# BICLab/Spike2Former

Measured on AMD Instinct MI355X. Metric: fwd+bwd images/sec, 512x512 T=4 ADE20K-150, higher is better.
Workload: dtype f32 (fp32-equivalent: bf16 hi+mid+lo split operands on bf16 MFMA, fp32 accumulate; spike maps stored as bf16, exact); 1 GPU; C2: 512x512 T=4 K=150 Meta-SpikeFormer [64, 128, 256, 360] + MaskFormer head, per-GPU batch 2; global_batch=2, parallelism=dp1, weights=random-init (name-seeded)

## Files before the change

spike2former_amd/csrc/dwconv.hip:

```cpp
#include "s2f_common.h"
#include <cstdlib>

#pragma clang fp contract(fast)

namespace {

constexpr int TS = 32;

__device__ __forceinline__ float ldx(const float* p) { return *p; }
__device__ __forceinline__ float ldx(const unsigned short* p) { return __uint_as_float(((unsigned int)*p) << 16); }
__device__ __forceinline__ float4 ldx4(const float* p) { return *reinterpret_cast<const float4*>(p); }
__device__ __forceinline__ float4 ldx4(const unsigned short* p) {
  const uint2 v = *reinterpret_cast<const uint2*>(p);
  return make_float4(__uint_as_float(v.x << 16), __uint_as_float(v.x & 0xffff0000u), __uint_as_float(v.y << 16),
                     __uint_as_float(v.y & 0xffff0000u));
}

template <int K, typename TX>
__device__ __forceinline__ void stage_halo(float (&s)[TS + K - 1][TS + K], const TX* __restrict__ xp, int H, int W, int oy0,
                                           int ox0, int po, float fillv, int fpad, bool vec_ok) {
  constexpr int HS = TS + K - 1;
  auto at = [&](int iy, int ix) -> float {
    if (iy >= 0 && iy < H && ix >= 0 && ix < W) return ldx(xp + (int64_t)iy * W + ix);
    if (iy >= -fpad && iy < H + fpad && ix >= -fpad && ix < W + fpad) return fillv;
    return 0.f;
  };
  {
    const int ri = threadIdx.x >> 3, qi = (threadIdx.x & 7) * 4;
    const int iy = oy0 + po + ri, ix = ox0 + po + qi;
    float4 v;
    if (vec_ok && iy >= 0 && iy < H && ix >= 0 && ix + 3 < W) {
      v = ldx4(xp + (int64_t)iy * W + ix);
    } else {
      v = make_float4(at(iy, ix), at(iy, ix + 1), at(iy, ix + 2), at(iy, ix + 3));
    }
    float* d = &s[po + ri][po + qi];
    d[0] = v.x; d[1] = v.y; d[2] = v.z; d[3] = v.w;
  }
  constexpr int RING = HS * HS - TS * TS;
  const int top = po * HS, bot = (K - 1 - po) * HS;
  for (int e = threadIdx.x; e < RING; e += 256) {
    int r, q;
    if (e < top) {
      r = e / HS; q = e - r * HS;
    } else if (e < top + bot) {
      const int f = e - top;
      r = po + TS + f / HS; q = f % HS;
    } else {
      const int f = e - top - bot;
      r = po + f / (K - 1);
      const int j = f % (K - 1);
      q = j < po ? j : TS + j;
    }
    s[r][q] = at(oy0 + r, ox0 + q);
  }
}

struct DwEpi {
  const float* mean;
  const float* var;
  const float* gamma;
  const float* beta;
  float* u_out;
  unsigned short* y;
  unsigned long long* stats;
  float eps, vth, Df, inv_d;
  float* part;
  int P;
};

__device__ __forceinline__ void dw_epi_store(const DwEpi& ep, int c, int64_t off, const float (&acc)[4], int nvalid, bool vec,
                                             uint32_t& csum, uint32_t& cnz) {
#pragma clang fp contract(off)
  const float mean = ep.mean[c], rstd = 1.0f / sqrtf(ep.var[c] + ep.eps), g = ep.gamma[c], be = ep.beta[c];
  float u[4], yy[4] = {0.f, 0.f, 0.f, 0.f};
#pragma unroll
  for (int o = 0; o < 4; ++o) {
    u[o] = (acc[o] - mean) * rstd * g + be;
    if (ep.y && o < nvalid) {
      float sp, vn;
      bool inr;
      s2f_lif_update(u[o], ep.Df, ep.inv_d, ep.vth, sp, yy[o], vn, inr);
      csum += (uint32_t)sp;
      cnz += ((uint32_t)sp != 0);
    }
  }
  if (vec && nvalid == 4) {
    if (ep.u_out) *reinterpret_cast<float4*>(ep.u_out + off) = make_float4(u[0], u[1], u[2], u[3]);
    if (ep.y) *reinterpret_cast<uint2*>(ep.y + off) = s2f_spikes_to_bf16x4(yy[0], yy[1], yy[2], yy[3]);
  } else {
#pragma unroll
    for (int o = 0; o < 4; ++o) {
      if (o >= nvalid) continue;
      if (ep.u_out) ep.u_out[off + o] = u[o];
      if (ep.y) ep.y[off + o] = (unsigned short)(__float_as_uint(yy[o]) >> 16);
    }
  }
}

__device__ __forceinline__ void dw_epi_counters(const DwEpi& ep, uint32_t csum, uint32_t cnz) {
  if (ep.y == nullptr || ep.stats == nullptr) return;
  for (int o = 32; o > 0; o >>= 1) {
    csum += __shfl_xor(csum, o, 64);
    cnz += __shfl_xor(cnz, o, 64);
  }
  if ((threadIdx.x & 63) == 0) {
    unsigned long long* slot = ep.stats + 2 * ((blockIdx.x * 4 + (threadIdx.x >> 6) + blockIdx.y * 7) % S2F_STAT_SLOTS);
    if (csum) atomicAdd(&slot[0], (unsigned long long)csum);
    if (cnz) atomicAdd(&slot[1], (unsigned long long)cnz);
  }
}

__device__ __forceinline__ void dw_tile_stats(const DwEpi& ep, int c, int n, float s1, float s2) {
  __shared__ float red[4][2];
  for (int o = 32; o > 0; o >>= 1) {
    s1 += __shfl_xor(s1, o, 64);
    s2 += __shfl_xor(s2, o, 64);
  }
  if ((threadIdx.x & 63) == 0) {
    red[threadIdx.x >> 6][0] = s1;
    red[threadIdx.x >> 6][1] = s2;
  }
  __syncthreads();
  if (threadIdx.x == 0) {
    const int64_t slot = (int64_t)c * ep.P + (int64_t)n * gridDim.x + blockIdx.x;
    *reinterpret_cast<float2*>(ep.part + slot * 2) =
        make_float2((red[0][0] + red[1][0]) + (red[2][0] + red[3][0]), (red[0][1] + red[1][1]) + (red[2][1] + red[3][1]));
  }
}

template <int K, bool FLIP, typename TX, bool EPI = false, bool STATS = false>
__global__ __launch_bounds__(256) void dw_stencil_kernel(const TX* __restrict__ x, const float* __restrict__ w,
                                                         const float* __restrict__ border, float* __restrict__ y, int C,
                                                         int H, int W, int Ho, int Wo, int pad, int tiles_x, DwEpi ep = DwEpi{}) {
  constexpr int HS = TS + K - 1;
  __shared__ float s[HS][HS + 1];
  const int plane = blockIdx.y;
  const int c = plane % C;
  const int ty = (blockIdx.x / tiles_x) * TS, tx = (blockIdx.x % tiles_x) * TS;
  const TX* xp = x + (int64_t)plane * H * W;
  const float fillv = (!FLIP && border) ? border[c] : 0.f;
  const int po = FLIP ? K - 1 - pad : pad;
  const bool vec_ok = (W & 3) == 0 && (reinterpret_cast<uintptr_t>(xp) & (4 * sizeof(TX) - 1)) == 0;
  stage_halo<K, TX>(s, xp, H, W, ty - po, tx - po, po, fillv, FLIP ? 0 : pad, vec_ok);
  float wk[K * K];
#pragma unroll
  for (int i = 0; i < K * K; ++i) wk[i] = w[c * K * K + i];
  __syncthreads();
  const int r = threadIdx.x >> 3;
  const int q0 = (threadIdx.x & 7) * 4;
  float acc[4] = {0.f, 0.f, 0.f, 0.f};
#pragma unroll
  for (int i = 0; i < K; ++i) {
    float row[K + 3];
#pragma unroll
    for (int j = 0; j < K + 3; ++j) row[j] = s[r + i][q0 + j];
#pragma unroll
    for (int j = 0; j < K; ++j) {
      const float wv = FLIP ? wk[(K - 1 - i) * K + (K - 1 - j)] : wk[i * K + j];
#pragma unroll
      for (int o = 0; o < 4; ++o) acc[o] += wv * row[j + o];
    }
  }
  const int oy = ty + r;
  if constexpr (EPI) {
    uint32_t csum = 0, cnz = 0;
    if (oy < Ho && tx + q0 < Wo) {
      const int64_t off = (int64_t)plane * Ho * Wo + (int64_t)oy * Wo + tx + q0;
      dw_epi_store(ep, c, off, acc, min(4, Wo - tx - q0), (Wo & 3) == 0 && (off & 3) == 0, csum, cnz);
    }
    dw_epi_counters(ep, csum, cnz);
    return;
  }
  if (oy < Ho) {
    float* yp = y + (int64_t)plane * Ho * Wo + (int64_t)oy * Wo + tx + q0;
    if ((Wo & 3) == 0 && tx + q0 + 3 < Wo && (reinterpret_cast<uintptr_t>(yp) & 15u) == 0) {
      *reinterpret_cast<float4*>(yp) = make_float4(acc[0], acc[1], acc[2], acc[3]);
    } else {
#pragma unroll
      for (int o = 0; o < 4; ++o)
        if (tx + q0 + o < Wo) yp[o] = acc[o];
    }
  }
  if constexpr (STATS) {
    float s1 = 0.f, s2 = 0.f;
#pragma unroll
    for (int o = 0; o < 4; ++o)
      if (oy < Ho && tx + q0 + o < Wo) {
        s1 += acc[o];
        s2 += acc[o] * acc[o];
      }
    dw_tile_stats(ep, c, plane / C, s1, s2);
  }
}

constexpr int WT = 64, HT = 32, WS = WT + 8;

template <int K, bool FLIP, typename TX, bool EPI = false, bool STATS = false>
__global__ __launch_bounds__(256) void dw_stencil_wide_kernel(const TX* __restrict__ x, const float* __restrict__ w,
                                                              const float* __restrict__ border, float* __restrict__ y,
                                                              int C, int H, int W, int Ho, int Wo, int pad, int tiles_x,
                                                              DwEpi ep = DwEpi{}) {
  constexpr int HR = HT + K - 1;
  __shared__ __attribute__((aligned(16))) float s[HR][WS];
  const int plane = blockIdx.y;
  const int c = plane % C;
  const int ty = (blockIdx.x / tiles_x) * HT, tx = (blockIdx.x % tiles_x) * WT;
  const TX* xp = x + (int64_t)plane * H * W;
  const float fillv = (!FLIP && border) ? border[c] : 0.f;
  const int po = pad;
  for (int e = threadIdx.x; e < HR * (WS / 4); e += 256) {
    const int r = e / (WS / 4), g = e - r * (WS / 4);
    const int iy = ty - po + r, ix = tx - 4 + g * 4;
    const bool in = iy >= 0 && iy < H && ix >= 0 && ix < W;
    const float4 v = ldx4(xp + (in ? (int64_t)iy * W + ix : 0));
    *reinterpret_cast<float4*>(&s[r][g * 4]) = in ? v : make_float4(fillv, fillv, fillv, fillv);
  }
  float wk[K * K];
#pragma unroll
  for (int i = 0; i < K * K; ++i) wk[i] = w[c * K * K + i];
  __syncthreads();
  const int r2 = (threadIdx.x >> 4) * 2;
  const int q0 = (threadIdx.x & 15) * 4;
  constexpr int SH = 4 - (K - 1) / 2;
  float acc[2][4] = {{0.f, 0.f, 0.f, 0.f}, {0.f, 0.f, 0.f, 0.f}};
#pragma unroll
  for (int i = 0; i < K + 1; ++i) {
    float row[12];
#pragma unroll
    for (int v4 = 0; v4 < 3; ++v4) {
      const float4 t = *reinterpret_cast<const float4*>(&s[r2 + i][q0 + v4 * 4]);
      row[v4 * 4] = t.x; row[v4 * 4 + 1] = t.y; row[v4 * 4 + 2] = t.z; row[v4 * 4 + 3] = t.w;
    }
#pragma unroll
    for (int a = 0; a < 2; ++a) {
      const int ki = i - a;
      if (ki < 0 || ki >= K) continue;
#pragma unroll
      for (int j = 0; j < K; ++j) {
        const float wv = FLIP ? wk[(K - 1 - ki) * K + (K - 1 - j)] : wk[ki * K + j];
#pragma unroll
        for (int o = 0; o < 4; ++o) acc[a][o] += wv * row[j + o + SH];
      }
    }
  }
  if constexpr (EPI) {
    uint32_t csum = 0, cnz = 0;
#pragma unroll
    for (int a = 0; a < 2; ++a) {
      const int oy = ty + r2 + a, ox = tx + q0;
      if (oy >= Ho || ox >= Wo) continue;
      const int64_t off = (int64_t)plane * Ho * Wo + (int64_t)oy * Wo + ox;
      dw_epi_store(ep, c, off, acc[a], min(4, Wo - ox), (Wo & 3) == 0 && (off & 3) == 0, csum, cnz);
    }
    dw_epi_counters(ep, csum, cnz);
    return;
  }
#pragma unroll
  for (int a = 0; a < 2; ++a) {
    const int oy = ty + r2 + a, ox = tx + q0;
    if (oy >= Ho) continue;
    float* yp = y + (int64_t)plane * Ho * Wo + (int64_t)oy * Wo + ox;
    if ((Wo & 3) == 0 && ox + 3 < Wo && (reinterpret_cast<uintptr_t>(yp) & 15u) == 0) {
      *reinterpret_cast<float4*>(yp) = make_float4(acc[a][0], acc[a][1], acc[a][2], acc[a][3]);
    } else {
#pragma unroll
      for (int o = 0; o < 4; ++o)
        if (ox + o < Wo) yp[o] = acc[a][o];
    }
  }
  if constexpr (STATS) {
    float s1 = 0.f, s2 = 0.f;
#pragma unroll
    for (int a = 0; a < 2; ++a)
#pragma unroll
      for (int o = 0; o < 4; ++o)
        if (ty + r2 + a < Ho && tx + q0 + o < Wo) {
          s1 += acc[a][o];
          s2 += acc[a][o] * acc[a][o];
        }
    dw_tile_stats(ep, c, plane / C, s1, s2);
  }
}

template <int K, typename TX>
__global__ __launch_bounds__(256) void dw_wgrad_kernel(const TX* __restrict__ x, const float* __restrict__ border,
                                                       const float* __restrict__ gy, float* __restrict__ gw, int C, int H,
                                                       int W, int Ho, int Wo, int pad, int tiles_x, int ntiles) {
  constexpr int HS = TS + K - 1;
  constexpr int KK = K * K;
  __shared__ float s[HS][HS + 1];
  __shared__ float red[4][KK];
  const int plane = blockIdx.y;
  const int c = plane % C;
  const TX* xp = x + (int64_t)plane * H * W;
  const float* gp = gy + (int64_t)plane * Ho * Wo;
  const float fillv = border ? border[c] : 0.f;
  const bool vec_ok = (W & 3) == 0 && (reinterpret_cast<uintptr_t>(xp) & (4 * sizeof(TX) - 1)) == 0;
  const int r = threadIdx.x >> 3, q0 = (threadIdx.x & 7) * 4;
  float acc[KK];
#pragma unroll
  for (int t = 0; t < KK; ++t) acc[t] = 0.f;
  for (int tile = blockIdx.x; tile < ntiles; tile += gridDim.x) {
    const int ty = (tile / tiles_x) * TS, tx = (tile % tiles_x) * TS;
    __syncthreads();
    stage_halo<K, TX>(s, xp, H, W, ty - pad, tx - pad, pad, fillv, pad, vec_ok);
    float g[4] = {0.f, 0.f, 0.f, 0.f};
    const int oy = ty + r, ox = tx + q0;
    const float* p = gp + (int64_t)oy * Wo + ox;
    if (oy < Ho) {
      if ((Wo & 3) == 0 && ox + 3 < Wo && (reinterpret_cast<uintptr_t>(p) & 15u) == 0) {
        const float4 v = *reinterpret_cast<const float4*>(p);
        g[0] = v.x; g[1] = v.y; g[2] = v.z; g[3] = v.w;
      } else {
#pragma unroll
        for (int o = 0; o < 4; ++o)
          if (ox + o < Wo) g[o] = p[o];
      }
    }
    __syncthreads();
#pragma unroll
    for (int i = 0; i < K; ++i) {
      float row[K + 3];
#pragma unroll
      for (int j = 0; j < K + 3; ++j) row[j] = s[r + i][q0 + j];
#pragma unroll
      for (int j = 0; j < K; ++j)
        acc[i * K + j] += (g[0] * row[j] + g[1] * row[j + 1]) + (g[2] * row[j + 2] + g[3] * row[j + 3]);
    }
  }
  const int lane = threadIdx.x & 63, wave = threadIdx.x >> 6;
#pragma unroll
  for (int t = 0; t < KK; ++t) {
    const float v = s2f_wave_sum_lane63(acc[t]);
    if (lane == 63) red[wave][t] = v;
  }
  __syncthreads();
  if (threadIdx.x < KK) {
    const float t = (red[0][threadIdx.x] + red[1][threadIdx.x]) + (red[2][threadIdx.x] + red[3][threadIdx.x]);
    atomicAdd(gw + c * KK + threadIdx.x, t);
  }
}

int check(const char* who, int N, int C, int H, int W, int K, int pad, int& Ho, int& Wo) {
  S2F_REQUIRE(N > 0 && C > 0 && H > 0 && W > 0, S2F_EINVAL, "%s: bad shape", who);
  S2F_REQUIRE(K == 3 || K == 5 || K == 7, S2F_EINVAL, "%s: kernel size %d not in {3,5,7}", who, K);
  S2F_REQUIRE(pad >= 0 && pad < K, S2F_EINVAL, "%s: bad padding %d", who, pad);
  Ho = H + 2 * pad - K + 1;
  Wo = W + 2 * pad - K + 1;
  S2F_REQUIRE(Ho > 0 && Wo > 0, S2F_EINVAL, "%s: empty output", who);
  S2F_REQUIRE((int64_t)N * C < 65536 * 16, S2F_EINVAL, "%s: too many planes", who);
  return S2F_OK;
}

constexpr int kStencilSizes[] = {3, 5, 7};
template <class F>
void for_stencil_size(int K, const F& launch) {
  s2f_dispatch<kStencilSizes>([&](int k) { return k == K; }, launch);
}

template <typename TX>
void launch_stencil_epi(int K, dim3 grid, hipStream_t s, const TX* x, const float* w, const float* border, int C, int H, int W, int Ho,
                        int Wo, int pad, int tiles_x, DwEpi ep) {
  if (K == 3 && (W & 3) == 0 && W >= 2 * WT && H >= HT && pad == 1 && (reinterpret_cast<uintptr_t>(x) & (4 * sizeof(TX) - 1)) == 0) {
    const int wx = (Wo + WT - 1) / WT, wy = (Ho + HT - 1) / HT;
    hipLaunchKernelGGL((dw_stencil_wide_kernel<3, false, TX, true>), dim3(wx * wy, grid.y), dim3(256), 0, s, x, w, border,
                       (float*)nullptr, C, H, W, Ho, Wo, pad, wx, ep);
    return;
  }
  for_stencil_size(K, [&](auto i) {
    hipLaunchKernelGGL((dw_stencil_kernel<kStencilSizes[i], false, TX, true>), grid, dim3(256), 0, s, x, w, border, (float*)nullptr,
                       C, H, W, Ho, Wo, pad, tiles_x, ep);
  });
}

inline bool wide_form(int K, int H, int W, int pad) {
  static const bool wide_on = !getenv("S2F_DW_NO_WIDE");
  return wide_on && K == 3 && (W & 3) == 0 && W >= 2 * WT && H >= HT && pad == 1;
}

inline int stats_tiles(int H, int W) {
  return wide_form(3, H, W, 1) ? ((W + WT - 1) / WT) * ((H + HT - 1) / HT) : ((W + TS - 1) / TS) * ((H + TS - 1) / TS);
}

template <typename TX>
void launch_stencil_stats(hipStream_t s, const TX* x, const float* w, float* y, float* part, int N, int C, int H, int W) {
  DwEpi ep{};
  ep.part = part;
  ep.P = N * stats_tiles(H, W);
  if (wide_form(3, H, W, 1)) {
    const int wx = (W + WT - 1) / WT, wy = (H + HT - 1) / HT;
    hipLaunchKernelGGL((dw_stencil_wide_kernel<3, false, TX, false, true>), dim3(wx * wy, N * C), dim3(256), 0, s, x, w,
                       (const float*)nullptr, y, C, H, W, H, W, 1, wx, ep);
    return;
  }
  const int tiles_x = (W + TS - 1) / TS, tiles_y = (H + TS - 1) / TS;
  hipLaunchKernelGGL((dw_stencil_kernel<3, false, TX, false, true>), dim3(tiles_x * tiles_y, N * C), dim3(256), 0, s, x, w,
                     (const float*)nullptr, y, C, H, W, H, W, 1, tiles_x, ep);
}

template <bool FLIP, typename TX>
void launch_stencil(int K, dim3 grid, hipStream_t s, const TX* x, const float* w, const float* border, float* y, int C,
                    int H, int W, int Ho, int Wo, int pad, int tiles_x) {
  if (wide_form(K, H, W, pad) && (reinterpret_cast<uintptr_t>(x) & (4 * sizeof(TX) - 1)) == 0) {
    const int wx = (Wo + WT - 1) / WT, wy = (Ho + HT - 1) / HT;
    hipLaunchKernelGGL((dw_stencil_wide_kernel<3, FLIP, TX>), dim3(wx * wy, grid.y), dim3(256), 0, s, x, w, border, y, C, H, W, Ho,
                       Wo, pad, wx, DwEpi{});
    return;
  }
  for_stencil_size(K, [&](auto i) {
    hipLaunchKernelGGL((dw_stencil_kernel<kStencilSizes[i], FLIP, TX>), grid, dim3(256), 0, s, x, w, border, y, C, H, W, Ho, Wo, pad,
                       tiles_x, DwEpi{});
  });
}

}

extern "C" int s2f_dwconv_fwd(const void* x, const float* w, const float* border, float* y, int N, int C, int H, int W,
                              int K, int pad, int x_bf16, void* stream) {
  S2F_REQUIRE(x && w && y, S2F_EINVAL, "s2f_dwconv_fwd: null pointer");
  int Ho, Wo;
  int rc = check("s2f_dwconv_fwd", N, C, H, W, K, pad, Ho, Wo);
  if (rc) return rc;
  const int tiles_x = (Wo + TS - 1) / TS, tiles_y = (Ho + TS - 1) / TS;
  if (x_bf16)
    launch_stencil<false>(K, dim3(tiles_x * tiles_y, N * C), (hipStream_t)stream, reinterpret_cast<const unsigned short*>(x), w,
                          border, y, C, H, W, Ho, Wo, pad, tiles_x);
  else
    launch_stencil<false>(K, dim3(tiles_x * tiles_y, N * C), (hipStream_t)stream, reinterpret_cast<const float*>(x), w, border,
                          y, C, H, W, Ho, Wo, pad, tiles_x);
  return s2f_check_launch("s2f_dwconv_fwd");
}

extern "C" int64_t s2f_dwconv_stats_slots(int N, int H, int W) {
  return (N > 0 && H > 0 && W > 0) ? (int64_t)N * stats_tiles(H, W) : 0;
}

extern "C" int s2f_dwconv_fwd_stats(const void* x, const float* w, float* y, float* partials, int64_t P, int N, int C, int H, int W,
                                    int x_bf16, void* stream) {
  S2F_REQUIRE(x && w && y && partials, S2F_EINVAL, "s2f_dwconv_fwd_stats: null pointer");
  int Ho, Wo;
  int rc = check("s2f_dwconv_fwd_stats", N, C, H, W, 3, 1, Ho, Wo);
  if (rc) return rc;
  S2F_REQUIRE(P == s2f_dwconv_stats_slots(N, H, W), S2F_EINVAL, "s2f_dwconv_fwd_stats: P must be s2f_dwconv_stats_slots(N, H, W)");
  S2F_REQUIRE((reinterpret_cast<uintptr_t>(x) & (x_bf16 ? 7u : 15u)) == 0 && (reinterpret_cast<uintptr_t>(partials) & 7u) == 0,
              S2F_EALIGN, "s2f_dwconv_fwd_stats: x must be aligned to four elements, partials to 8 bytes");
  if (x_bf16)
    launch_stencil_stats((hipStream_t)stream, reinterpret_cast<const unsigned short*>(x), w, y, partials, N, C, H, W);
  else
    launch_stencil_stats((hipStream_t)stream, reinterpret_cast<const float*>(x), w, y, partials, N, C, H, W);
  return s2f_check_launch("s2f_dwconv_fwd_stats");
}

extern "C" int s2f_dwconv_bn_lif_fwd(const void* x, const float* w, const float* border, const float* running_mean,
                                     const float* running_var, const float* gamma, const float* beta, float eps, float* u_out,
                                     void* y_bf16, uint64_t* stats, int N, int C, int H, int W, int K, int pad, int x_bf16, float vth,
                                     int D, void* stream) {
  S2F_REQUIRE(x && w && running_mean && running_var && gamma && beta && (u_out || y_bf16), S2F_EINVAL,
              "s2f_dwconv_bn_lif_fwd: null pointer / neither output requested");
  S2F_REQUIRE(!y_bf16 || s2f_bf16_spikes_exact(D), S2F_EINVAL, "s2f_dwconv_bn_lif_fwd: bf16 spikes need D a power of two <= 128");
  int Ho, Wo;
  int rc = check("s2f_dwconv_bn_lif_fwd", N, C, H, W, K, pad, Ho, Wo);
  if (rc) return rc;
  const int tiles_x = (Wo + TS - 1) / TS, tiles_y = (Ho + TS - 1) / TS;
  DwEpi ep{running_mean, running_var, gamma, beta, u_out, reinterpret_cast<unsigned short*>(y_bf16),
           reinterpret_cast<unsigned long long*>(stats), eps, vth, (float)D, 1.0f / (float)D};
  if (x_bf16)
    launch_stencil_epi(K, dim3(tiles_x * tiles_y, N * C), (hipStream_t)stream, reinterpret_cast<const unsigned short*>(x), w, border, C,
                       H, W, Ho, Wo, pad, tiles_x, ep);
  else
    launch_stencil_epi(K, dim3(tiles_x * tiles_y, N * C), (hipStream_t)stream, reinterpret_cast<const float*>(x), w, border, C, H, W,
                       Ho, Wo, pad, tiles_x, ep);
  return s2f_check_launch("s2f_dwconv_bn_lif_fwd");
}

extern "C" int s2f_dwconv_bwd_input(const float* gy, const float* w, float* gx, int N, int C, int H, int W, int K, int pad,
                                    void* stream) {
  S2F_REQUIRE(gy && w && gx, S2F_EINVAL, "s2f_dwconv_bwd_input: null pointer");
  int Ho, Wo;
  int rc = check("s2f_dwconv_bwd_input", N, C, H, W, K, pad, Ho, Wo);
  if (rc) return rc;
  const int tiles_x = (W + TS - 1) / TS, tiles_y = (H + TS - 1) / TS;
  launch_stencil<true>(K, dim3(tiles_x * tiles_y, N * C), (hipStream_t)stream, gy, w, nullptr, gx, C, Ho, Wo, H, W, pad,
                       tiles_x);
  return s2f_check_launch("s2f_dwconv_bwd_input");
}

extern "C" int s2f_dwconv_bwd_weight(const void* x_in, const float* border, const float* gy, float* gw, int N, int C, int H,
                                     int W, int K, int pad, int accumulate, int x_bf16, void* stream) {
  S2F_REQUIRE(x_in && gy && gw, S2F_EINVAL, "s2f_dwconv_bwd_weight: null pointer");
  int Ho, Wo;
  int rc = check("s2f_dwconv_bwd_weight", N, C, H, W, K, pad, Ho, Wo);
  if (rc) return rc;
  hipStream_t s = (hipStream_t)stream;
  if (!accumulate && s2f_zero_async(gw, sizeof(float) * (size_t)C * K * K, s) != S2F_OK)
    return s2f_check_launch("s2f_dwconv_bwd_weight memset");
  const int tiles_x = (Wo + TS - 1) / TS, tiles_y = (Ho + TS - 1) / TS;
  const int ntiles = tiles_x * tiles_y;
  int per_plane = (8192 + N * C - 1) / (N * C);
  if (per_plane > ntiles) per_plane = ntiles;
  if (per_plane < 1) per_plane = 1;
  const dim3 grid(per_plane, N * C);
  for_stencil_size(K, [&](auto i) {
    s2f_dispatch_bool(x_bf16 != 0, [&](auto bf) {
      using TX = std::conditional_t<bf.value, unsigned short, float>;
      hipLaunchKernelGGL((dw_wgrad_kernel<kStencilSizes[i], TX>), grid, dim3(256), 0, s, reinterpret_cast<const TX*>(x_in), border,
                         gy, gw, C, H, W, Ho, Wo, pad, tiles_x, ntiles);
    });
  });
  return s2f_check_launch("s2f_dwconv_bwd_weight");
}
```

Baseline: 58.19 images/s.

## Add row-pair interleaved depthwise conv kernels for K=5/7 forward and weight grad

Adds stencil and weight-gradient kernels that stage input rows into shared memory as interleaved row pairs. Each thread can then issue packed two-wide FMAs over adjacent output rows, which cuts shared-memory reads and FMA instruction count per output. The forward path uses them for K=5/7 (K=3 keeps the wide kernel). The weight-gradient path uses them for all kernel sizes that meet alignment and shape conditions, with larger tiles and a smaller grid. It adds more template code and depends on alignment checks; the shared-memory tile geometry (WS/HT/WT) is reused from the wide kernel.

```diff
diff --git a/spike2former_amd/csrc/dwconv.hip b/spike2former_amd/csrc/dwconv.hip
--- a/spike2former_amd/csrc/dwconv.hip
+++ b/spike2former_amd/csrc/dwconv.hip
@@ -283,6 +283,151 @@
   }
 }
 
+typedef float f2 __attribute__((ext_vector_type(2)));
+typedef float f4 __attribute__((ext_vector_type(4)));
+
+template <int NP, typename TX>
+__device__ __forceinline__ void stage_pairs(f2 (&s)[NP][WS], const TX* __restrict__ xp, int H, int W, int iy0, int tx, float fillv) {
+  constexpr int G = WS / 4, RP = 256 / G, IT = (NP + RP - 1) / RP;
+  const int p0 = threadIdx.x / G, g = threadIdx.x - p0 * G;
+  const int ix = tx - 4 + g * 4;
+  const bool inx = p0 < RP && ix >= 0 && ix < W;
+  float4 a[IT], b[IT];
+#pragma unroll
+  for (int k = 0; k < IT; ++k) {
+    const int p = p0 + RP * k, iy = iy0 + p;
+    const bool in0 = inx && p < NP && iy >= 0 && iy < H, in1 = inx && p < NP && iy + 1 >= 0 && iy + 1 < H;
+    a[k] = ldx4(xp + (in0 ? (int64_t)iy * W + ix : 0));
+    b[k] = ldx4(xp + (in1 ? (int64_t)(iy + 1) * W + ix : 0));
+    if (!in0) a[k] = make_float4(fillv, fillv, fillv, fillv);
+    if (!in1) b[k] = make_float4(fillv, fillv, fillv, fillv);
+  }
+#pragma unroll
+  for (int k = 0; k < IT; ++k) {
+    const int p = p0 + RP * k;
+    if (p0 >= RP || p >= NP) continue;
+    f4* d = reinterpret_cast<f4*>(&s[p][g * 4]);
+    d[0] = f4{a[k].x, b[k].x, a[k].y, b[k].y};
+    d[1] = f4{a[k].z, b[k].z, a[k].w, b[k].w};
+  }
+}
+
+__device__ __forceinline__ void read_pairs(f2 (&row)[12], const f2* __restrict__ srow) {
+#pragma unroll
+  for (int v = 0; v < 6; ++v) {
+    const f4 t = *reinterpret_cast<const f4*>(srow + 2 * v);
+    row[2 * v] = f2{t.x, t.y};
+    row[2 * v + 1] = f2{t.z, t.w};
+  }
+}
+
+template <int K, bool FLIP, typename TX>
+__global__ __launch_bounds__(256) void dw_stencil_pair_kernel(const TX* __restrict__ x, const float* __restrict__ w,
+                                                              const float* __restrict__ border, float* __restrict__ y, int C,
+                                                              int H, int W, int Ho, int Wo, int pad, int tiles_x) {
+  constexpr int NP = HT + K - 2;
+  constexpr int SH = 4 - (K - 1) / 2;
+  __shared__ __attribute__((aligned(16))) f2 s[NP][WS];
+  const int plane = blockIdx.y;
+  const int c = plane % C;
+  const int ty = (blockIdx.x / tiles_x) * HT, tx = (blockIdx.x % tiles_x) * WT;
+  const TX* xp = x + (int64_t)plane * H * W;
+  const float fillv = (!FLIP && border) ? border[c] : 0.f;
+  stage_pairs<NP, TX>(s, xp, H, W, ty - pad, tx, fillv);
+  float wk[K * K];
+#pragma unroll
+  for (int i = 0; i < K * K; ++i) wk[i] = w[c * K * K + i];
+  __syncthreads();
+  const int r2 = (threadIdx.x >> 4) * 2;
+  const int q0 = (threadIdx.x & 15) * 4;
+  f2 acc[4] = {f2{0.f, 0.f}, f2{0.f, 0.f}, f2{0.f, 0.f}, f2{0.f, 0.f}};
+#pragma unroll
+  for (int i = 0; i < K; ++i) {
+    f2 row[12];
+    read_pairs(row, &s[r2 + i][q0]);
+#pragma unroll
+    for (int j = 0; j < K; ++j) {
+      const float wv = FLIP ? wk[(K - 1 - i) * K + (K - 1 - j)] : wk[i * K + j];
+#pragma unroll
+      for (int o = 0; o < 4; ++o) acc[o] = __builtin_elementwise_fma(f2{wv, wv}, row[j + o + SH], acc[o]);
+    }
+  }
+#pragma unroll
+  for (int a = 0; a < 2; ++a) {
+    const int oy = ty + r2 + a, ox = tx + q0;
+    if (oy >= Ho) continue;
+    float* yp = y + (int64_t)plane * Ho * Wo + (int64_t)oy * Wo + ox;
+    if ((Wo & 3) == 0 && ox + 3 < Wo && (reinterpret_cast<uintptr_t>(yp) & 15u) == 0) {
+      *reinterpret_cast<float4*>(yp) = make_float4(acc[0][a], acc[1][a], acc[2][a], acc[3][a]);
+    } else {
+#pragma unroll
+      for (int o = 0; o < 4; ++o)
+        if (ox + o < Wo) yp[o] = acc[o][a];
+    }
+  }
+}
+
+template <int K, typename TX>
+__global__ __launch_bounds__(256) void dw_wgrad_pair_kernel(const TX* __restrict__ x, const float* __restrict__ border,
+                                                            const float* __restrict__ gy, float* __restrict__ gw, int C, int H,
+                                                            int W, int Ho, int Wo, int pad, int tiles_x, int ntiles) {
+  constexpr int KK = K * K;
+  constexpr int NI = (K + 1) / 2;
+  constexpr int NP = HT + K - 1;
+  constexpr int SH = 4 - (K - 1) / 2;
+  __shared__ __attribute__((aligned(16))) f2 s[NP][WS];
+  __shared__ float red[4][KK];
+  const int plane = blockIdx.y;
+  const int c = plane % C;
+  const TX* xp = x + (int64_t)plane * H * W;
+  const float* gp = gy + (int64_t)plane * Ho * Wo;
+  const float fillv = border ? border[c] : 0.f;
+  const int r = threadIdx.x >> 4, q0 = (threadIdx.x & 15) * 4;
+  f2 acc[NI][K];
+#pragma unroll
+  for (int ip = 0; ip < NI; ++ip)
+#pragma unroll
+    for (int j = 0; j < K; ++j) acc[ip][j] = f2{0.f, 0.f};
+  for (int tile = blockIdx.x; tile < ntiles; tile += gridDim.x) {
+    const int ty = (tile / tiles_x) * HT, tx = (tile % tiles_x) * WT;
+    __syncthreads();
+    float4 g[2];
+#pragma unroll
+    for (int a = 0; a < 2; ++a) {
+      const int oy = ty + r + 16 * a, ox = tx + q0;
+      const bool in = oy < Ho && ox < Wo;
+      g[a] = *reinterpret_cast<const float4*>(gp + (in ? (int64_t)oy * Wo + ox : 0));
+      if (!in) g[a] = make_float4(0.f, 0.f, 0.f, 0.f);
+    }
+    stage_pairs<NP, TX>(s, xp, H, W, ty - pad, tx, fillv);
+    __syncthreads();
+#pragma unroll
+    for (int a = 0; a < 2; ++a) {
+      const float gv[4] = {g[a].x, g[a].y, g[a].z, g[a].w};
+#pragma unroll
+      for (int ip = 0; ip < NI; ++ip) {
+        f2 row[12];
+        read_pairs(row, &s[r + 16 * a + 2 * ip][q0]);
+#pragma unroll
+        for (int j = 0; j < K; ++j)
+#pragma unroll
+          for (int o = 0; o < 4; ++o) acc[ip][j] = __builtin_elementwise_fma(f2{gv[o], gv[o]}, row[j + o + SH], acc[ip][j]);
+      }
+    }
+  }
+  const int lane = threadIdx.x & 63, wave = threadIdx.x >> 6;
+#pragma unroll
+  for (int t = 0; t < KK; ++t) {
+    const float v = s2f_wave_sum_lane63(acc[(t / K) >> 1][t % K][(t / K) & 1]);
+    if (lane == 63) red[wave][t] = v;
+  }
+  __syncthreads();
+  if (threadIdx.x < KK) {
+    const float t = (red[0][threadIdx.x] + red[1][threadIdx.x]) + (red[2][threadIdx.x] + red[3][threadIdx.x]);
+    atomicAdd(gw + c * KK + threadIdx.x, t);
+  }
+}
+
 template <int K, typename TX>
 __global__ __launch_bounds__(256) void dw_wgrad_kernel(const TX* __restrict__ x, const float* __restrict__ border,
                                                        const float* __restrict__ gy, float* __restrict__ gw, int C, int H,
@@ -383,6 +528,11 @@
   return wide_form(3, H, W, 1) ? ((W + WT - 1) / WT) * ((H + HT - 1) / HT) : ((W + TS - 1) / TS) * ((H + TS - 1) / TS);
 }
 
+inline bool pair_form(int K, int H, int W, int pad) {
+  static const bool pair_on = !getenv("S2F_DW_NO_PAIR");
+  return pair_on && pad == (K - 1) / 2 && (W & 3) == 0 && W >= WT && H >= HT;
+}
+
 template <typename TX>
 void launch_stencil_stats(hipStream_t s, const TX* x, const float* w, float* y, float* part, int N, int C, int H, int W) {
   DwEpi ep{};
@@ -406,6 +556,16 @@
     const int wx = (Wo + WT - 1) / WT, wy = (Ho + HT - 1) / HT;
     hipLaunchKernelGGL((dw_stencil_wide_kernel<3, FLIP, TX>), dim3(wx * wy, grid.y), dim3(256), 0, s, x, w, border, y, C, H, W, Ho,
                        Wo, pad, wx, DwEpi{});
+    return;
+  }
+  if (K != 3 && pair_form(K, H, W, pad) && (reinterpret_cast<uintptr_t>(x) & (4 * sizeof(TX) - 1)) == 0) {
+    const int wx = (Wo + WT - 1) / WT, wy = (Ho + HT - 1) / HT;
+    if (K == 5)
+      hipLaunchKernelGGL((dw_stencil_pair_kernel<5, FLIP, TX>), dim3(wx * wy, grid.y), dim3(256), 0, s, x, w, border, y, C, H, W, Ho, Wo,
+                         pad, wx);
+    else
+      hipLaunchKernelGGL((dw_stencil_pair_kernel<7, FLIP, TX>), dim3(wx * wy, grid.y), dim3(256), 0, s, x, w, border, y, C, H, W, Ho, Wo,
+                         pad, wx);
     return;
   }
   for_stencil_size(K, [&](auto i) {
@@ -495,15 +655,23 @@
   hipStream_t s = (hipStream_t)stream;
   if (!accumulate && s2f_zero_async(gw, sizeof(float) * (size_t)C * K * K, s) != S2F_OK)
     return s2f_check_launch("s2f_dwconv_bwd_weight memset");
-  const int tiles_x = (Wo + TS - 1) / TS, tiles_y = (Ho + TS - 1) / TS;
+  const bool pair = pair_form(K, H, W, pad) && (reinterpret_cast<uintptr_t>(x_in) & (x_bf16 ? 7u : 15u)) == 0 &&
+                    (reinterpret_cast<uintptr_t>(gy) & 15u) == 0;
+  const int tw = pair ? WT : TS, th = pair ? HT : TS;
+  const int tiles_x = (Wo + tw - 1) / tw, tiles_y = (Ho + th - 1) / th;
   const int ntiles = tiles_x * tiles_y;
-  int per_plane = (8192 + N * C - 1) / (N * C);
+  int per_plane = ((pair ? 2048 : 8192) + N * C - 1) / (N * C);
   if (per_plane > ntiles) per_plane = ntiles;
   if (per_plane < 1) per_plane = 1;
   const dim3 grid(per_plane, N * C);
   for_stencil_size(K, [&](auto i) {
     s2f_dispatch_bool(x_bf16 != 0, [&](auto bf) {
       using TX = std::conditional_t<bf.value, unsigned short, float>;
+      if (pair) {
+        hipLaunchKernelGGL((dw_wgrad_pair_kernel<kStencilSizes[i], TX>), grid, dim3(256), 0, s, reinterpret_cast<const TX*>(x_in),
+                           border, gy, gw, C, H, W, Ho, Wo, pad, tiles_x, ntiles);
+        return;
+      }
       hipLaunchKernelGGL((dw_wgrad_kernel<kStencilSizes[i], TX>), grid, dim3(256), 0, s, reinterpret_cast<const TX*>(x_in), border,
                          gy, gw, C, H, W, Ho, Wo, pad, tiles_x, ntiles);
     });
```

New measurement: 58.60 images/s, median of 6. No clear change (+0.7%).
